# pascalPost/turbomesh

Hardware: AMD Instinct MI355X
Metric: nodes smoothed/sec (elliptic sweeps, 4096^2 blocks) + achieved HBM GB/s (higher is better)
Workload: dtype f64

## Files before the change

turbomesh_amd/csrc/tm_api.cpp:

```cpp
#include "tm_smoother.hpp"
#include <cmath>
#include <cstdlib>
#include <cstring>
#include <limits>
#include <memory>

using namespace tmh;

#include "tm_api_util.hpp"
#include "tm_ilu.hpp"
#include "tm_refine.hpp"
#include "tm_quality_dev.hpp"

static void require_gfx950() {
    static int checked = 0;
    if (checked) return;
    int dev = 0;
    HIPCHK(hipGetDevice(&dev));
    hipDeviceProp_t prop;
    HIPCHK(hipGetDeviceProperties(&prop, dev));
    if (std::strncmp(prop.gcnArchName, "gfx950", 6) != 0)
        throw TmError(TM_E_HIP, std::string("libtm_hip is built for gfx950 (MI355X) only, found ") + prop.gcnArchName);
    checked = 1;
}
// ... 596 lines not shown
            shape[4 * l + 2] = L[l].ci;
            shape[4 * l + 3] = L[l].cj;
        }
        if (cycle) {
            cycle[0] = h.nu_pre;
            cycle[1] = h.nu_post;
            cycle[2] = h.nu_coarsest;
            cycle[3] = m.mg_dirichlet ? 1 : 0;
            cycle[4] = m.mg_perimeter_step ? 1 : 0;
            cycle[5] = m.mg_perimeter_sweeps;
        }
        if (omega) *omega = h.omega;
        return TM_OK;
    });
}
int tm_smoother_precondition_probe(tm_smoother* s, const double* f, double* z, double* f_after) {
    return guarded([&]() {
        if (!s || !f || !z) throw TmError(TM_E_ARG, "null argument");
        s->impl.precondition_probe_host(f, z, f_after);
        return TM_OK;
    });
}

int tm_smoother_queue_ordering(const tm_smoother* s) { return s ? s->impl.queue_ordering : static_cast<int>(TM_E_ARG); }

int tm_smooth_mesh(const tm_mesh_desc* mesh, uint64_t iterations, const tm_solver_opt* opt, const tm_control_fn* cf, tm_stats* stats) {
    tm_smoother* h = nullptr;
    int rc = tm_smoother_create(mesh, opt, cf, nullptr, nullptr, &h);
    if (rc < 0) return rc;
    tm_stats st;
    std::memset(&st, 0, sizeof(st));
    rc = tm_smoother_iterate(h, iterations, &st);
    if (rc >= 0 && iterations > 0) {
        const int rd = tm_smoother_download(h, mesh);
        if (rd < 0) rc = rd;
    }
    tm_smoother_destroy(h);
    if (stats) *stats = st;
    return rc;
}

int tm_plan_local(const tm_mesh_desc* mesh, const int32_t* owner, int32_t rank, int32_t nranks, tm_plan_local_info* out) {
    return guarded([&]() {
        if (!mesh || !owner || !out) throw TmError(TM_E_ARG, "null argument");
        std::memset(out, 0, sizeof(*out));
        const Topology t = topo_of(mesh);
// ... 184 lines not shown
```

turbomesh_amd/csrc/tm_kernels.h:

```cpp
#pragma once
#include <hip/hip_runtime.h>
#include <cstdint>
#include "tm_edge_types.h"
#include <vector>

namespace tmh {

enum ApplyMode : int {
    MODE_RAW = 0,
    MODE_SCALED = 1,
    MODE_RESID = 2,
    MODE_RELAX = 3,
    MODE_DIAG_COPY = 4,
    MODE_DIAG_SUM9 = 5,
    MODE_DIAG_NOSTORE = 6,
    MODE_DIAG_NOLOAD = 7,
    MODE_DIAG_MATH = 8,
    MODE_MG_RESID = 9,
    MODE_MG_SMOOTH = 10,
    MODE_MG_FIRST2 = 11
};
enum DotMode : int {
    DOT_NONE = 0,
    DOT_AUX = 1,
// ... 205 lines not shown
};
hipError_t launch_white(const WhiteArgs& w, int update, hipStream_t stream);

struct MgPair {
    int nif, njf, nic, njc;
    int ci, cj;
};
hipError_t launch_mg_inject(const double2* fine, double2* coarse, const MgPair& g, double scale_x, double scale_y, hipStream_t stream);
hipError_t launch_mg_restrict(const double2* r_fine, const double2* X_coarse, double2* f_coarse, const MgPair& g, hipStream_t stream);
hipError_t launch_mg_prolong_smooth(const ApplyBlock& a, const MgPair& g, hipStream_t stream);
struct MgPairArgs {
    const double2* in = nullptr;
    const double2* xk = nullptr;
    const double2* pq = nullptr;
    const double2* f = nullptr;
    double2* out = nullptr;
    double2* out2 = nullptr;
    const double2* coarse = nullptr;
    const double2* xc = nullptr;
    double2* fc = nullptr;
    int nic = 0, njc = 0, ci = 0, cj = 0;
    int ni = 0, nj = 0;
    double omega = 1.0;
};
bool mg_pair_supported(int ni, int nj);
bool mg_pair_restrict_supported(int ni, int nj, int ci, int cj);
hipError_t launch_mg_pair(const MgPairArgs& a, int kind, hipStream_t stream);
hipError_t launch_mg_prolong_add(const double2* e_coarse, double2* e_fine, const MgPair& g, hipStream_t stream);
hipError_t launch_mg_scale(const double2* f, double2* out, int ni, int nj, double omega, hipStream_t stream);

hipError_t launch_soa_planes(const double2* in, double* plane0, double* plane1, int ni, int nj, hipStream_t stream);

hipError_t launch_debug_white_math(const double* x, const double* y, uint64_t n, double* out_acos, double* out_atan2, hipStream_t stream);

}
```

turbomesh_amd/csrc/tm_kernels.hip:

```cpp
#include "tm_kernels.h"
#include "tm_devutil.hpp"
#include "tm_refmath.h"
#include <cstdlib>
#include <type_traits>

namespace tmh {

__device__ __forceinline__ double lane_prev(double edge, double v) {
    int2 o = __builtin_bit_cast(int2, edge), s = __builtin_bit_cast(int2, v), r;
    r.x = __builtin_amdgcn_update_dpp(o.x, s.x, 0x138 , 0xf, 0xf, false);
    r.y = __builtin_amdgcn_update_dpp(o.y, s.y, 0x138, 0xf, 0xf, false);
    return __builtin_bit_cast(double, r);
}
__device__ __forceinline__ double lane_next(double edge, double v) {
    int2 o = __builtin_bit_cast(int2, edge), s = __builtin_bit_cast(int2, v), r;
    r.x = __builtin_amdgcn_update_dpp(o.x, s.x, 0x130 , 0xf, 0xf, false);
    r.y = __builtin_amdgcn_update_dpp(o.y, s.y, 0x130, 0xf, 0xf, false);
    return __builtin_bit_cast(double, r);
}
__device__ __forceinline__ double2 lane_prev(double2 edge, double2 v) { return make_double2(lane_prev(edge.x, v.x), lane_prev(edge.y, v.y)); }
__device__ __forceinline__ double2 lane_next(double2 edge, double2 v) { return make_double2(lane_next(edge.x, v.x), lane_next(edge.y, v.y)); }

__device__ __forceinline__ double2 lane_prev0(double2 v) {
    int4 s = __builtin_bit_cast(int4, v), r;
// ... 985 lines not shown
template <bool HAS_PQ>
__device__ __forceinline__ double2 mg_scaled_row(const MgMetric& g, const Row3& m, const Row3& c, const Row3& p, double P, double Q) {
    double ax = p.c.x + m.c.x, ay = p.c.y + m.c.y;
    double bx = c.h.x, by = c.h.y;
    if (HAS_PQ) {
        const double hP = 0.5 * P, hQ = 0.5 * Q;
        ax = fma(hP, p.c.x - m.c.x, ax);
        ay = fma(hP, p.c.y - m.c.y, ay);
        bx = fma(hQ, c.e.x, bx);
        by = fma(hQ, c.e.y, by);
    }
    const double kx = p.e.x - m.e.x;
    const double ky = p.e.y - m.e.y;
    double sx = g.G22 * ax, sy = g.G22 * ay;
    sx = fma(g.G11, bx, sx);
    sy = fma(g.G11, by, sy);
    sx = fma(g.m2D, c.c.x, sx);
    sy = fma(g.m2D, c.c.y, sy);
    sx = fma(g.mhG12, kx, sx);
    sy = fma(g.mhG12, ky, sy);
    return make_double2(sx * g.rinv, sy * g.rinv);
}

template <int KIND, bool HAS_PQ, bool PRO, bool RST, int U>
__device__ __forceinline__ void mg_pair_strip(const MgPairArgs& a, const Relax2Tile& t) {
    static_assert(!RST || KIND == 1, "the restriction rides behind the residual");
    const int ni = a.ni, nj = a.nj;
    const int cc = min(max(t.c, 0), nj - 1);
    const double2 zero = make_double2(0.0, 0.0);
    auto at = [&](int row) { return static_cast<size_t>(min(max(row, 0), ni - 1)) * nj + cc; };
    const bool perim_col = (t.c <= 0) || (t.c >= nj - 1);
    const bool col_in = (t.c >= 1) && (t.c <= nj - 2);
    const int nrows = t.i1 - t.i0;
    const __amdgpu_buffer_rsrc_t out_rsrc = __builtin_amdgcn_make_buffer_rsrc(a.out + static_cast<size_t>(t.i0) * nj, 0, nrows * nj * 16, 0x00020000);
    const __amdgpu_buffer_rsrc_t out2_rsrc =
        __builtin_amdgcn_make_buffer_rsrc((KIND == 1 ? a.out2 : a.out) + static_cast<size_t>(t.i0) * nj, 0, nrows * nj * 16, 0x00020000);
    const unsigned lane_off = static_cast<unsigned>(cc) * 16u;
    const int cj1 = PRO ? min(a.cj ? ((cc + 1) >> 1) : cc, a.njc - 1) : 0;
    const bool midway = PRO && a.cj && (cc & 1);

    struct Ld {
        double2 in, x, f, pq, c0, c1;
    };
    auto load_step = [&](int i, Ld& L) {
        const size_t ar = at(i + 2), aq = at(i + 1);
        L.in = a.in[ar];
        L.x = a.xk[ar];
        if (KIND == 0) L.f = a.f[aq];
        if (HAS_PQ) L.pq = a.pq[aq];
        if (PRO) {
            const int r = min(max(i + 2, 0), ni - 1);
            const int ci0 = min(a.ci ? (r >> 1) : r, a.nic - 1), ci1 = min(a.ci ? ((r + 1) >> 1) : r, a.nic - 1);
            const double2* r0 = a.coarse + static_cast<size_t>(ci0) * a.njc;
            const double2* r1 = a.coarse + static_cast<size_t>(ci1) * a.njc;
            L.c0 = r0[cj1];
            L.c1 = r1[cj1];
        }
    };
    auto entering = [&](int row, const Ld& L) {
        if (KIND == 1) return (col_in && row >= 1 && row <= ni - 2) ? L.in : zero;
        if (!PRO) return L.in;
        const double2 l0 = lane_prev0(L.c0), l1 = lane_prev0(L.c1);
        const double2 a0 = midway ? l0 : L.c0, a1 = midway ? l1 : L.c1;
        const double2 v = make_double2(L.in.x + 0.25 * ((a0.x + L.c0.x) + (a1.x + L.c1.x)), L.in.y + 0.25 * ((a0.y + L.c0.y) + (a1.y + L.c1.y)));
        return (col_in && row >= 1 && row <= ni - 2) ? v : L.in;
    };
    auto det_of = [&](double2 x) { return sub2(lane_next0(x), lane_prev0(x)); };

    Row3 A[3], S[3];
    double2 Xc[3], Xe_cur;
    MgMetric Mp = {0.0, 0.0, 0.0, 0.0, 0.0, 0.0};
    double2 f_prev = zero, pq_prev = zero;
    double2 rm2 = zero, rm1 = zero;
    Ld cur[U], nxt[U];
    {
        Ld w0, w1;
        load_step(t.i0 - 4, w0);
        load_step(t.i0 - 3, w1);
#pragma unroll
        for (int u = 0; u < U; ++u) load_step(t.i0 - 2 + u, cur[u]);
        A[0] = make_row(entering(t.i0 - 2, w0));
        A[1] = make_row(entering(t.i0 - 1, w1));
        Xc[0] = w0.x;
        Xc[1] = w1.x;
        Xe_cur = det_of(w1.x);
        A[2].c = A[2].e = A[2].h = zero;
        S[0] = S[1] = S[2] = A[2];
        Xc[2] = zero;
    }
    const int nsteps = nrows + (RST ? 3 : 2);
    auto group = [&](const int tb) {
#pragma unroll
        for (int u = 0; u < U; ++u) load_step(t.i0 - 2 + tb + U + u, nxt[u]);
#pragma unroll
        for (int u = 0; u < U; ++u) {
            const int A0 = u % 3, A1 = (u + 1) % 3, A2 = (u + 2) % 3;
            const Ld& L = cur[u];
            const int i = t.i0 - 2 + tb + u;
            const int q = i + 1;
            A[A2] = make_row(entering(i + 2, L));
            Xc[A2] = L.x;
            const double2 Xe_next = det_of(L.x);
            const MgMetric M = mg_metric(sub2(Xc[A2], Xc[A0]), Xe_cur);
            const double2 t1 = mg_scaled_row<HAS_PQ>(M, A[A0], A[A1], A[A2], HAS_PQ ? L.pq.x : 0.0, HAS_PQ ? L.pq.y : 0.0);
            const double2 fq = (KIND == 0) ? L.f : A[A1].c;
            double2 s1;
            if (KIND == 0) {
                const double2 res = sub2(fq, t1);
                s1 = make_double2(fma(a.omega, res.x, A[A1].c.x), fma(a.omega, res.y, A[A1].c.y));
            } else {
                s1 = make_double2(a.omega * fma(-a.omega, t1.x, 2.0 * A[A1].c.x), a.omega * fma(-a.omega, t1.y, 2.0 * A[A1].c.y));
            }
            const bool perim_row = (q <= 0) || (q >= ni - 1);
            if (perim_row || perim_col) s1 = zero;
            if (KIND == 1) {
                const bool own = t.out_lane && !perim_row && (q >= t.i0) && (q < t.i1);
                __builtin_amdgcn_raw_buffer_store_b128(__builtin_bit_cast(v4i32, s1), out_rsrc,
                                                       static_cast<int>(own ? lane_off + static_cast<unsigned>((q - t.i0) * nj * 16) : OOB_VOFFSET), 0, 0);
            }
            S[A2] = make_row(s1);
            const double2 t2 = mg_scaled_row<HAS_PQ>(Mp, S[A0], S[A1], S[A2], HAS_PQ ? pq_prev.x : 0.0, HAS_PQ ? pq_prev.y : 0.0);
// ... 19 lines not shown
                        acc.y = fma(wi * 0.25, l.y, acc.y);
                        acc.x = fma(wi * 0.5, v.x, acc.x);
                        acc.y = fma(wi * 0.5, v.y, acc.y);
                        acc.x = fma(wi * 0.25, r.x, acc.x);
                        acc.y = fma(wi * 0.25, r.y, acc.y);
                    };
                    row_sum(rm2, 0.25);
                    row_sum(rm1, 0.5);
                    row_sum(oz, 0.25);
                    const int ci = (i - 1) >> 1, cj = t.c >> 1, lane = t.c - t.c0 + 2;
                    const bool emit = !(t.c & 1) && lane >= 4 && lane <= 60 && t.c >= 2 && t.c <= nj - 2 && ci >= 1 && ci <= a.nic - 2 && cj <= a.njc - 2;
                    if (emit) {
                        const size_t oc = static_cast<size_t>(ci) * a.njc + cj;
                        const double2 xp = a.xc[oc + a.njc], xm = a.xc[oc - a.njc], xr = a.xc[oc + 1], xl = a.xc[oc - 1];
                        const double dxx = xp.x - xm.x, dxy = xp.y - xm.y, dex = xr.x - xl.x, dey = xr.y - xl.y;
                        const double aic = -0.5 * (fma(dxx, dxx, dxy * dxy) + fma(dex, dex, dey * dey));
                        const double k = 16.0 / ((aic == 0.0) ? 1.0 : aic);
                        a.fc[oc] = make_double2(k * acc.x, k * acc.y);
                    }
                }
                rm2 = rm1;
                rm1 = oz;
            }
            Mp = M;
            f_prev = fq;
            if (HAS_PQ) pq_prev = L.pq;
            Xe_cur = Xe_next;
        }
#pragma unroll
        for (int u = 0; u < U; ++u) cur[u] = nxt[u];
    };
    group(0);
    for (int tb = U; tb < nsteps; tb += U) group(tb);
}

template <int KIND, bool HAS_PQ, bool PRO, bool RST = false>
__global__ __launch_bounds__(256) void k_mg_pair(MgPairArgs a, int RI, int nSG, int nRC) {
    const int lane = threadIdx.x & 63;
    const int wave = threadIdx.x >> 6;
    const int total = nSG * nRC, bid = blockIdx.x;
    const int q8 = total >> 3, rem = total & 7, xcd = bid & 7, k8 = bid >> 3;
    const int logical = (xcd < rem) ? xcd * (q8 + 1) + k8 : rem * (q8 + 1) + (xcd - rem) * q8 + k8;
    const int rc = logical / nSG;
    const int sg = logical - rc * nSG;
    Relax2Tile t;
    t.c0 = (sg * 4 + wave) * (RST ? MG_RST_W : 60);
    t.c = t.c0 - 2 + lane;
    t.out_lane = (lane >= (RST ? 3 : 2)) && (lane <= (RST ? 60 : 61)) && (t.c >= 1) && (t.c <= a.nj - 2);
    t.i0 = 1 + rc * RI;
    t.i1 = min(t.i0 + RI, a.ni - 1);
    if (t.c0 + (RST ? 1 : 0) <= a.nj - 2 && t.i0 < t.i1) mg_pair_strip<KIND, HAS_PQ, PRO, RST, 3>(a, t);
}

bool mg_pair_supported(int ni, int nj) { return ni >= 5 && nj >= 5 && nj <= (1 << 20); }
bool mg_pair_restrict_supported(int ni, int nj, int ci, int cj) {
    if (!mg_pair_supported(ni, nj) || !ci || !cj) return false;
    const int nstrips = (nj - 2 + MG_RST_W - 1) / MG_RST_W, nSG = (nstrips + 3) / 4;
    return static_cast<long>(nSG) * ((ni - 2 + 17) / 18) >= 1024;
}
hipError_t launch_mg_pair(const MgPairArgs& a, int kind, hipStream_t st) {
    if (!mg_pair_supported(a.ni, a.nj)) return hipErrorInvalidValue;
    if (kind == 1 && a.fc) {
        if (!mg_pair_restrict_supported(a.ni, a.nj, a.ci, a.cj) || !a.xc) return hipErrorInvalidValue;
        const int nstrips = (a.nj - 2 + MG_RST_W - 1) / MG_RST_W, nSG = (nstrips + 3) / 4, RI = 18, nRC = (a.ni - 2 + RI - 1) / RI;
        const dim3 grid(nSG * nRC), block(256);
        if (a.pq) hipLaunchKernelGGL((k_mg_pair<1, true, false, true>), grid, block, 0, st, a, RI, nSG, nRC);
        else hipLaunchKernelGGL((k_mg_pair<1, false, false, true>), grid, block, 0, st, a, RI, nSG, nRC);
        return hipGetLastError();
    }
    const int nstrips = (a.nj - 1 + 59) / 60, nSG = (nstrips + 3) / 4, interior = a.ni - 2;
    int RI = 18;
    while (RI > 3 && static_cast<long>(nSG) * ((interior + RI - 1) / RI) < 1024) RI -= 3;
    RI = std::max(1, std::min(RI, interior));
    const int nRC = (interior + RI - 1) / RI;
    const dim3 grid(nSG * nRC), block(256);
    const bool pq = a.pq != nullptr, pro = a.coarse != nullptr;
    if (kind == 1) {
        if (pq) hipLaunchKernelGGL((k_mg_pair<1, true, false>), grid, block, 0, st, a, RI, nSG, nRC);
        else hipLaunchKernelGGL((k_mg_pair<1, false, false>), grid, block, 0, st, a, RI, nSG, nRC);
    } else if (pro) {
        if (pq) hipLaunchKernelGGL((k_mg_pair<0, true, true>), grid, block, 0, st, a, RI, nSG, nRC);
        else hipLaunchKernelGGL((k_mg_pair<0, false, true>), grid, block, 0, st, a, RI, nSG, nRC);
    } else {
        if (pq) hipLaunchKernelGGL((k_mg_pair<0, true, false>), grid, block, 0, st, a, RI, nSG, nRC);
// ... 1616 lines not shown
```

turbomesh_amd/csrc/tm_multigrid.cpp:

```cpp
#include "tm_multigrid.hpp"
#include "tm_smoother.hpp"

#include <algorithm>
#include <cmath>
#include <cstdio>
#include <cstdlib>

namespace tmh {

#define HIPCHK(x) hip_check((x), #x)

static void log_aspect_stats(const double* xy, int ni, int nj, double& mean, double& sdev) {
    mean = sdev = 0.0;
    if (!xy || ni < 3 || nj < 3) return;
    const int si = std::max(1, (ni - 2) / 64), sj = std::max(1, (nj - 2) / 64);
    double sum = 0.0, sum2 = 0.0;
    long cnt = 0;
    for (int i = 1; i < ni - 1; i += si)
        for (int j = 1; j < nj - 1; j += sj) {
            const double* c = xy + 2 * (static_cast<size_t>(i) * nj + j);
            const double ax = c[2 * nj] - c[-2 * nj], ay = c[2 * nj + 1] - c[-2 * nj + 1];
            const double bx = c[2] - c[-2], by = c[3] - c[-1];
            const double g11 = ax * ax + ay * ay, g22 = bx * bx + by * by;
            if (g11 > 0.0 && g22 > 0.0) {
// ... 105 lines not shown
    a.aux = f;
    a.out = out;
    a.ni = l.ni;
    a.nj = l.nj;
    a.omega = omega;
    a.partials = nullptr;
    HIPCHK(launch_apply_block(a, MODE_MG_SMOOTH, DOT_NONE, st));
}

void BlockMG::residual(const MgLevel& l, const double2* f, const double2* in, double2* out, hipStream_t st) const {
    ApplyBlock a;
    a.in = in;
    a.xk = l.X;
    a.pq = l.PQ;
    a.aux = f;
    a.out = out;
    a.ni = l.ni;
    a.nj = l.nj;
    a.omega = 0.0;
    a.partials = nullptr;
    HIPCHK(launch_apply_block(a, MODE_MG_RESID, DOT_NONE, st));
}

void BlockMG::vcycle(const double2* f0, double2* z, double2* w0, double2* w1, hipStream_t st) {
    const size_t nl = L.size();
    std::vector<double2*> cur(nl, nullptr), oth(nl, nullptr);
    std::vector<const double2*> rhs(nl, nullptr);
    const int pre_extra = nu_pre > 0 ? nu_pre - 1 : 0;
    auto pair_ok = [&](size_t l) { return use_pair && mg_pair_supported(L[l].ni, L[l].nj); };
    const bool pair_pre0 = pair_ok(0) && nu_pre == 2 && nl > 1, pair_post0 = pair_ok(0) && nu_post == 2;
    (void)pair_pre0;
    const int flips0 = (nl == 1) ? pre_extra + nu_coarsest : pre_extra + (pair_post0 ? 1 : nu_post);
    cur[0] = (flips0 % 2 == 0) ? z : w0;
    oth[0] = (flips0 % 2 == 0) ? w0 : z;
    rhs[0] = f0;
    L[0].r = w1;
    for (size_t l = 1; l < nl; ++l) {
        cur[l] = L[l].a;
        oth[l] = L[l].b;
        rhs[l] = L[l].f;
    }
    auto sweeps = [&](size_t l, int n) {
        for (int k = 0; k < n; ++k) {
            smooth(L[l], rhs[l], cur[l], oth[l], st);
            std::swap(cur[l], oth[l]);
        }
    };
    for (size_t l = 0; l < nl; ++l) {
// ... 51 lines not shown
            sweeps(l, nu_coarsest);
            break;
        }
        residual(L[l], rhs[l], cur[l], L[l].r, st);
        HIPCHK(launch_mg_restrict(L[l].r, L[l + 1].X, L[l + 1].f, pair(l), st));
    }
    for (size_t l = nl - 1; l-- > 0;) {
        if (nu_post == 2 && pair_ok(l)) {
            MgPairArgs a;
            a.in = cur[l];
            a.xk = L[l].X;
            a.pq = L[l].PQ;
            a.f = rhs[l];
            a.out = oth[l];
            a.coarse = cur[l + 1];
            const MgPair g = pair(l);
            a.nic = g.nic;
            a.njc = g.njc;
            a.ci = g.ci;
            a.cj = g.cj;
            a.ni = L[l].ni;
            a.nj = L[l].nj;
            a.omega = omega;
            HIPCHK(launch_mg_pair(a, 0, st));
            std::swap(cur[l], oth[l]);
            continue;
        }
        if (fuse_prolong && nu_post >= 1 && static_cast<int64_t>(L[l].ni) * L[l].nj >= fuse_prolong_min) {
            ApplyBlock a;
            a.in = cur[l];
            a.in2 = cur[l + 1];
            a.xk = L[l].X;
            a.pq = L[l].PQ;
            a.aux = rhs[l];
            a.out = oth[l];
            a.ni = L[l].ni;
            a.nj = L[l].nj;
            a.omega = omega;
            a.partials = nullptr;
            HIPCHK(launch_mg_prolong_smooth(a, pair(l), st));
            std::swap(cur[l], oth[l]);
            sweeps(l, nu_post - 1);
        } else {
            HIPCHK(launch_mg_prolong_add(cur[l + 1], cur[l], pair(l), st));
            sweeps(l, nu_post);
        }
// ... 6 lines not shown
```

turbomesh_amd/csrc/tm_multigrid.hpp:

```cpp
#pragma once
#include "tm_kernels.h"
#include <vector>

namespace tmh {

class DeviceArena;

struct MgLevel {
    int ni = 0, nj = 0;
    int ci = 0, cj = 0;
    double2 *X = nullptr, *PQ = nullptr;
    double2 *f = nullptr, *a = nullptr, *b = nullptr, *r = nullptr;
};

class BlockMG {
   public:
    int nu_pre = 2, nu_post = 2, nu_coarsest = 8;
    int64_t fuse_prolong_min = 262144;
    bool fuse_prolong = true;
    double omega = 0.8;
    bool fuse_restrict = true;
    bool use_pair = true;
    void build(DeviceArena& arena, int ni, int nj, bool has_pq, double aspect, bool worst_case);
    static double aspect_of(const double* xy, int ni, int nj);
    static double aspect_spread_of(const double* xy, int ni, int nj);
    void set_field(const double2* X0, const double2* PQ0, hipStream_t stream);
    void vcycle(const double2* f, double2* z, double2* w0, double2* w1, hipStream_t stream);
    size_t nlevels() const { return L.size(); }
    const std::vector<MgLevel>& levels() const { return L; }

   private:
    std::vector<MgLevel> L;
    void smooth(const MgLevel& l, const double2* f, const double2* in, double2* out, hipStream_t st) const;
    void residual(const MgLevel& l, const double2* f, const double2* in, double2* out, hipStream_t st) const;
    MgPair pair(size_t fine) const;
};

}
```

turbomesh_amd/csrc/tm_smoother.cpp:

```cpp
#include "tm_smoother.hpp"
#include "tm_api_util.hpp"
#include "tm_ilu.hpp"
#include "tm_refine.hpp"
#include "tm_quality_dev.hpp"
#include <algorithm>
#include <atomic>
#include <chrono>
#include <cmath>
#include <cstdio>
#include <cstdlib>
#include <cstring>
#include <map>
#include <unordered_map>

namespace tmh {

void hip_check(hipError_t e, const char* what) {
    if (e != hipSuccess) throw TmError(TM_E_HIP, std::string(what) + ": " + hipGetErrorString(e));
}
#define HIPCHK(x) hip_check((x), #x)

std::atomic<int> g_multirank_handles{0};
tm_log_fn g_log_sink = nullptr;
void* g_log_ctx = nullptr;
// ... 430 lines not shown
            border_ids.push_back(static_cast<const int32_t*>(upload_table(ids.data(), ids.size() * 4)));
        }
        poff2_edge = off2;
        nwg_apply2 = off2 + edge_nf.nwg;
    }
    pipelined_single = fuse_pairs && !(has_hooks && (lp.send_ids.size() > 0 || !lp.ghost_gid.empty())) && edge_nf.nrows > 0 && lp.n_owned >= (1 << 21);
    if (const char* e = std::getenv("TM_SINGLE_PIPELINED")) pipelined_single = pipelined_single && std::atoi(e) != 0;
    fuse_triples = fuse_pairs && edge_nf.nrows == 0 && !(has_hooks && (!lp.send_ids.empty() || !lp.ghost_gid.empty()));
    if (const char* e = std::getenv("TM_FUSE_3")) fuse_triples = fuse_triples && std::atoi(e) != 0;
    if (fuse_triples || triples_coupled) {
        poff3.clear();
        rows3.clear();
        int off3 = 0;
        rows3 = relax3_rows_of_owned_blocks();
        for (size_t k = 0; k < lp.owned_blocks.size(); ++k) {
            const int64_t b = lp.owned_blocks[k];
            const int bi = static_cast<int>(topo.ni[b]), bj = static_cast<int>(topo.nj[b]);
            if (!relax3_supported(bi, bj)) fuse_triples = false;
            poff3.push_back(off3);
            off3 += relax3_block_nwg(bi, bj, rows3[k]);
        }
        nwg_apply3 = off3;
    }
    nwg_vec = vec_nwg(n_owned);
    const int nwg3_all = fuse_triples ? nwg_apply3 : (triples_coupled ? nwg_apply3 + std::max(edge_L[2].nwg, fused_levels.nstrips) : 0);
    if (vk_overlap) {
        int off_ov = 0;
        for (int64_t b : lp.owned_blocks) {
            poff_ov.push_back(off_ov);
            off_ov += apply_block_nwg_overlap(static_cast<int>(topo.ni[b]), static_cast<int>(topo.nj[b]), apply_rows);
        }
        poff_edge_ov = off_ov;
        nwg_apply_ov = off_ov + edge.nwg;
    }
    if (vk_able && std::max(nwg_apply, nwg_apply_ov) <= 512) nwg_vec = std::min(nwg_vec, 512);
    lazy = !has_hooks && opt.inner != TM_INNER_RELAX && std::max(std::max(nwg_apply, nwg_apply_ov), nwg_vec) <= 512 && !(opt.flags & TM_OPT_EAGER_SCALARS);
    const int nwg_refine = refine() ? csr_nwg(n_owned) : 0;
    const uint64_t npart = static_cast<uint64_t>(std::max(std::max(std::max(std::max(std::max(nwg_apply, nwg_apply_ov), nwg_apply2), nwg3_all), nwg_vec), nwg_refine)) * MAX_PARTIALS;
    fuse_s = !has_hooks && opt.inner == TM_INNER_BICGSTAB && !(opt.flags & TM_OPT_EAGER_SCALARS);
    fuse_p = fuse_s;
    if (const char* e = std::getenv("TM_FUSE_P")) fuse_p = fuse_p && std::atoi(e) != 0;
    fuse2 = fuse_p;
    if (const char* e = std::getenv("TM_FUSE_2")) fuse2 = fuse2 && std::atoi(e) != 0;
    if (fuse_p) {
        p_alt = vec();
        v_alt = vec();
    }
    if (fuse2) r_alt = vec();
    const int rows = static_cast<int>(npart / MAX_PARTIALS);
    const struct {
        const char* what;
        int nwg;
    } producers[] = {{"operator", nwg_apply},
                     {"operator (overlapping strips)", nwg_apply_ov},
                     {"sweep pairs", nwg_apply2},
                     {"sweep triples", nwg3_all},
                     {"vector kernels", nwg_vec},
                     {"GMRES Gram-Schmidt", (opt.inner == TM_INNER_GMRES || reference()) ? vec_nwg(n_owned) : 0},
                     {"perimeter-row right-hand side", opt.inner != TM_INNER_RELAX ? edge.nwg : 0},
                     {"refinement step", nwg_refine}};
    if (std::getenv("TM_DEBUG_RUNS"))
        std::fprintf(stderr, "[tm] partial-sum rows: %d allocated; operator %d, overlapping strips %d, pairs %d, triples %d, vector kernels %d (vec_nwg %d)\n", rows,
                     nwg_apply, nwg_apply_ov, nwg_apply2, nwg3_all, nwg_vec, vec_nwg(n_owned));
    for (const auto& q : producers)
        if (q.nwg > rows)
            throw TmError(TM_E_HIP, std::string("internal: the ") + q.what + " launch has " + std::to_string(q.nwg) + " workgroups, the partial-sum buffer " +
                                        std::to_string(rows) + " rows");
    return npart;
}

void Smoother::alloc_reductions(uint64_t npart) {
    partials_guard = false;
    if (const char* e = std::getenv("TM_PARTIALS_GUARD")) partials_guard = std::atoi(e) != 0;
    const uint64_t nguard = partials_guard ? GUARD_DOUBLES : 0;
    for (int k = 0; k < (lazy ? 3 : 1); ++k) part_buf[k] = arena.alloc_n<double>(npart + nguard);
    partials = part_buf[0];
    red = arena.alloc_n<double>(MAX_PARTIALS + nguard);
    if (partials_guard) {
        for (int k = 0; k < 3; ++k) guard[k] = part_buf[k] ? part_buf[k] + npart : nullptr;
        guard[3] = red ? red + MAX_PARTIALS : nullptr;
    }
    S_buf[0] = arena.alloc_n<KrylovScalars>(1);
    S_buf[1] = lazy ? arena.alloc_n<KrylovScalars>(1) : S_buf[0];
// ... 319 lines not shown
}

void Smoother::white_launch(int update) {
    WhiteArgs w;
    const auto idx = [&](int64_t b) { return lp.local_start[std::lower_bound(lp.owned_blocks.begin(), lp.owned_blocks.end(), b) - lp.owned_blocks.begin()]; };
    w.x0 = X + idx(0);
    w.x1 = X + idx(1);
    w.pq0 = PQ + idx(0);
    w.pq1 = PQ + idx(1);
    w.ni0 = static_cast<int>(topo.ni[0]);
    w.nj0 = static_cast<int>(topo.nj[0]);
    w.ni1 = static_cast<int>(topo.ni[1]);
    w.nj1 = static_cast<int>(topo.nj[1]);
    w.le_p0 = static_cast<int>(white_le.position[0]);
    w.le_p1 = static_cast<int>(white_le.position[1]);
    w.le_fi0 = static_cast<int>(white_le.first_internal[0]);
    w.le_fi1 = static_cast<int>(white_le.first_internal[1]);
    w.le_dir0 = static_cast<int>(white_le.direction[0]);
    w.ds_target = cf.ds_target;
    w.theta_target = cf.theta_target;
    HIPCHK(launch_white(w, update, stream));
}

void Smoother::precondition(const double2* in, double2* out) {
    double2* const in_w = const_cast<double2*>(in);
    const size_t nb = lp.owned_blocks.size(), ns = mg_streams.size();
    auto dims = [&](size_t k, int& bi, int& bj) {
        const int64_t b = lp.owned_blocks[k];
        bi = static_cast<int>(topo.ni[b]);
        bj = static_cast<int>(topo.nj[b]);
    };
    int bi, bj;
    if (mg_dirichlet)
        for (size_t k = 0; k < nb; ++k) {
            dims(k, bi, bj);
            const int64_t ls = lp.local_start[k];
            HIPCHK(launch_ring_dirichlet(in_w + ls, X + ls, PQ ? PQ + ls : nullptr, t + ls, bi, bj, stream));
        }
    if (ns > 1) HIPCHK(hipEventRecord(mg_fork, stream));
    for (size_t k = 0; k < nb; ++k) {
        const int64_t ls = lp.local_start[k];
        hipStream_t q = ns > 1 ? mg_streams[k % ns] : stream;
        if (ns > 1 && k < ns) HIPCHK(hipStreamWaitEvent(q, mg_fork, 0));
        mg[k].vcycle(in + ls, out + ls, mg_w0 + ls, mg_w1 + ls, q);
    }
    for (size_t q = 0; q < ns && ns > 1; ++q) {
        HIPCHK(hipEventRecord(mg_join[q], mg_streams[q]));
        HIPCHK(hipStreamWaitEvent(stream, mg_join[q], 0));
    }
    for (size_t k = 0; k < nb; ++k) {
        dims(k, bi, bj);
        const int64_t ls = lp.local_start[k];
        if (mg_dirichlet) HIPCHK(launch_ring_restore(in_w + ls, t + ls, bi, bj, stream));
        if (!mg_perimeter_step) HIPCHK(launch_copy_perimeter(in + ls, out + ls, bi, bj, stream));
    }
    if (!mg_perimeter_step) return;
    for (int sweep = 0; sweep < mg_perimeter_sweeps; ++sweep) {
        if (has_hooks) {
            exchange(out);
            exchange_finish();
        }
        HIPCHK(launch_edge_rows(edge, out, X, PQ, nullptr, t, 0.0, MODE_SCALED, DOT_NONE, nullptr, stream));
        for (size_t k = 0; k < lp.owned_blocks.size(); ++k) {
            const int64_t b = lp.owned_blocks[k];
            const int64_t ls = lp.local_start[k];
            HIPCHK(launch_perimeter_sub(in + ls, t + ls, out + ls, static_cast<int>(topo.ni[b]), static_cast<int>(topo.nj[b]), stream));
        }
    }
}

void Smoother::precondition_probe_host(const double* f, double* z, double* f_after) {
    if (!use_mg) throw TmError(TM_E_UNSUPPORTED, "tm_smoother_precondition_probe needs a handle created with TM_INNER_MG_BICGSTAB");
    if (has_hooks) throw TmError(TM_E_UNSUPPORTED, "tm_smoother_precondition_probe is available on single-process handles only");
    for (size_t k = 0; k < lp.owned_blocks.size(); ++k) mg[k].set_field(X + lp.local_start[k], PQ ? PQ + lp.local_start[k] : nullptr, stream);
    HIPCHK(hipMemcpyAsync(p, f, sizeof(double2) * n_owned, hipMemcpyHostToDevice, stream));
    precondition(p, p_hat);
    HIPCHK(hipMemcpyAsync(z, p_hat, sizeof(double2) * n_owned, hipMemcpyDeviceToHost, stream));
    if (f_after) HIPCHK(hipMemcpyAsync(f_after, p, sizeof(double2) * n_owned, hipMemcpyDeviceToHost, stream));
    sync();
}

int Smoother::poll_done(uint64_t it, bool final) {
    auto verdict = [&](const KrylovScalars* h, uint64_t at) {
        if (h->done[0] && h->done[1]) return (h->done[0] == 1 && h->done[1] == 1) ? 1 : 2;
        bool progress = false;
        for (int c = 0; c < 2; ++c) {
            if (h->done[c]) continue;
            if (!(stall_best[c] > 0.0) || h->rr[c] < 0.25 * stall_best[c]) {
                stall_best[c] = h->rr[c];
                progress = true;
            }
        }
        if (progress) stall_since = at;
        else if (at > stall_since && at - stall_since > stall_window) {
            stalled = true;
            return 2;
        }
        return 0;
    };
    flush_pending();
    if (!pipelined_poll) {
        HIPCHK(hipMemcpyAsync(h_S, S, sizeof(KrylovScalars), hipMemcpyDeviceToHost, stream));
// ... 67 lines not shown
                apply_virtual(VK_R, r, v, t, p_alt, v_alt, p, r_alt, U);
                std::swap(r, r_alt);
                std::swap(p, p_alt);
                std::swap(v, v_alt);
                apply_virtual(VK_S2, r, v, nullptr, nullptr, t);
                st.operator_sweeps += 2;
                it_total += 1;
                if (it_total % opt.check_every == 0 || it_total == opt.max_inner) {
                    const int verdict = poll_done(it_total, it_total == opt.max_inner);
                    if (verdict) {
                        converged = verdict == 1;
                        breakdown = !converged;
                        break;
                    }
                }
                continue;
            }
            if (fuse_p) {
                apply_virtual(VK_P, r, p, v, p_alt, v_alt);
                std::swap(p, p_alt);
                std::swap(v, v_alt);
            } else {
                HIPCHK(launch_p_update(scalars_for(), r, p, v, n_owned, nwg_vec, stream));
                if (use_mg) {
                    precondition(p, p_hat);
                    apply(p_hat, v, MODE_SCALED, DOT_AUX, r_hat, X, 0.0, STEP_SIGMA);
                } else {
                    apply(p, v, MODE_SCALED, DOT_AUX, r_hat, X, 0.0, STEP_SIGMA);
                }
            }
            if (fuse_s) {
                apply_virtual(VK_S, r, v, nullptr, nullptr, t);
                HIPCHK(launch_xr_update_vs(scalars_for(), U, p, v, t, r, r_hat, n_owned, nwg_vec, partials, stream));
                reduce_update(nwg_vec, STEP_RHO);
                st.operator_sweeps += 2;
                it_total += 1;
                if (it_total % opt.check_every == 0 || it_total == opt.max_inner) {
                    const int verdict = poll_done(it_total, it_total == opt.max_inner);
                    if (verdict) {
                        converged = verdict == 1;
                        breakdown = !converged;
                        break;
                    }
                }
                continue;
            }
            HIPCHK(launch_s_update(scalars_for(), r, v, s, n_owned, nwg_vec, partials, stream));
            reduce_update(nwg_vec, STEP_SS);
            if (use_mg) {
                precondition(s, s_hat);
                apply(s_hat, t, MODE_SCALED, DOT_AUX2, s, X, 0.0, STEP_TSTT);
            } else {
                apply(s, t, MODE_SCALED, DOT_IN, nullptr, X, 0.0, STEP_TSTT);
            }
            HIPCHK(launch_xr_update(scalars_for(), U, use_mg ? p_hat : p, use_mg ? s_hat : s, s, t, r, r_hat, n_owned, nwg_vec, partials, stream));
            reduce_update(nwg_vec, STEP_RHO);
            st.operator_sweeps += 2;
            it_total += 1;
            if (it_total % opt.check_every == 0 || it_total == opt.max_inner) {
                const int verdict = poll_done(it_total, it_total == opt.max_inner);
                if (verdict) {
                    converged = verdict == 1;
                    breakdown = !converged;
                    break;
                }
            }
        }
        if (fuse2) {
            flush_pending();
            HIPCHK(launch_xr_update_vs(scalars_for(), U, p, v, t, r, r_hat, n_owned, nwg_vec, partials, stream));
        }
        if (converged || !breakdown || stalled || restarts >= 8 || it_total >= opt.max_inner) break;
// ... 943 lines not shown
```

turbomesh_amd/csrc/tm_smoother.hpp:

```cpp
#pragma once
#include "../../include/tm_hip.h"
#include <cstdlib>
#include "tm_edge_tables.hpp"
#include "tm_kernels.h"
#include "tm_multigrid.hpp"
#include "tm_plan.hpp"
#include <cmath>
#include <atomic>
#include <memory>
#include <string>
#include <functional>
#include <vector>

namespace tmh {

struct TmError : std::runtime_error {
    int code;
    TmError(int c, const std::string& m) : std::runtime_error(m), code(c) {}
};
void hip_check(hipError_t e, const char* what);
extern std::atomic<int> g_multirank_handles;
extern tm_log_fn g_log_sink;
extern void* g_log_ctx;

// ... 26 lines not shown
    Topology topo;
    std::vector<PlanRow> all_rows;
    LocalPlan lp;
    tm_solver_opt opt{};
    tm_control_fn cf{};
    tm_comm_hooks hooks{};
    bool has_hooks = false;
    std::vector<int32_t> owner;
    hipStream_t stream = nullptr;
    DeviceArena arena;

    int64_t n_owned = 0, n_local = 0, n_ghost = 0, dof_global = 0;
    double2 *X = nullptr, *U = nullptr, *r = nullptr, *r_hat = nullptr, *p = nullptr, *v = nullptr, *s = nullptr, *t = nullptr;
    double2 *PQ = nullptr, *tmpA = nullptr, *tmpB = nullptr;
    double2 *p_hat = nullptr, *s_hat = nullptr, *mg_w0 = nullptr, *mg_w1 = nullptr;
    std::vector<BlockMG> mg;
    bool use_mg = false;
    bool mg_perimeter_step = false;
    bool mg_dirichlet = false;
    std::vector<hipStream_t> mg_streams;
    std::vector<hipEvent_t> mg_join;
    hipEvent_t mg_fork = nullptr;
    int mg_perimeter_sweeps = 2;
    void precondition(const double2* in, double2* out);
    void precondition_probe_host(const double* f, double* z, double* f_after);
    double2* M = nullptr;
    double2* M2 = nullptr;
    bool fuse_pairs = false;
    bool relax2_store_nt = true;
    bool pair_sync_events = false;
    size_t inside_lds = 0;
    EdgeRowsDev edge;
    std::vector<double> h_rhs;
    struct RhsTable {
        double* dev = nullptr;
        std::vector<const double*> src;
    };
    std::vector<RhsTable> rhs_tables;
    EdgeRowsDev edge_nf;
    EdgeRowsDev edge_nf_g;
    std::vector<int> dyn_mask;
    std::vector<const int32_t*> border_ids;
    std::vector<int> border_n;
    void prefill_fixed();
    double* partials = nullptr;
    double* red = nullptr;
    KrylovScalars* S = nullptr;
// ... 196 lines not shown
```

Baseline: 447.5 billion.

## Fold the scaled operator application and dot into the last multigrid post-smoothing pair

The final fine-level post-smoothing pair kernel now also applies the scaled operator to the freshly smoothed correction. It writes v/t and accumulates the DOT_AUX/AUX2 partial sums in the same strip pass, with a third row of lag. The perimeter rows are handled by an edge-rows launch, and one reduction covers both. This removes a separate full-grid read of z and write of v per BiCGSTAB half-step. The cost is heavier per-strip register use, narrower strips, and a gating condition on block size and hierarchy shape.

```diff
diff --git a/turbomesh_amd/csrc/tm_api.cpp b/turbomesh_amd/csrc/tm_api.cpp
--- a/turbomesh_amd/csrc/tm_api.cpp
+++ b/turbomesh_amd/csrc/tm_api.cpp
@@ -642,6 +642,16 @@
     });
 }
 
+#ifdef TM_DEBUG_EXPORTS
+int tm_debug_mg_fold_probe(tm_smoother* s, int branch, int folded, const double* f, const double* aux, double* z, double* v, double* sums) {
+    return guarded([&]() {
+        if (!s || !f || !aux || !z || !v || !sums || branch < 0 || branch > 1) throw TmError(TM_E_ARG, "bad argument");
+        s->impl.fold_probe_host(branch, folded != 0, f, aux, z, v, sums);
+        return TM_OK;
+    });
+}
+#endif
+
 int tm_smoother_queue_ordering(const tm_smoother* s) { return s ? s->impl.queue_ordering : static_cast<int>(TM_E_ARG); }
 
 int tm_smooth_mesh(const tm_mesh_desc* mesh, uint64_t iterations, const tm_solver_opt* opt, const tm_control_fn* cf, tm_stats* stats) {
diff --git a/turbomesh_amd/csrc/tm_kernels.h b/turbomesh_amd/csrc/tm_kernels.h
--- a/turbomesh_amd/csrc/tm_kernels.h
+++ b/turbomesh_amd/csrc/tm_kernels.h
@@ -251,8 +251,13 @@
     int nic = 0, njc = 0, ci = 0, cj = 0;
     int ni = 0, nj = 0;
     double omega = 1.0;
+    double2* vout = nullptr;
+    const double2* aux = nullptr;
+    double* partials = nullptr;
+    int dot = DOT_NONE;
 };
 bool mg_pair_supported(int ni, int nj);
+int mg_pair_apply_nwg(int ni, int nj);
 bool mg_pair_restrict_supported(int ni, int nj, int ci, int cj);
 hipError_t launch_mg_pair(const MgPairArgs& a, int kind, hipStream_t stream);
 hipError_t launch_mg_prolong_add(const double2* e_coarse, double2* e_fine, const MgPair& g, hipStream_t stream);
diff --git a/turbomesh_amd/csrc/tm_kernels.hip b/turbomesh_amd/csrc/tm_kernels.hip
--- a/turbomesh_amd/csrc/tm_kernels.hip
+++ b/turbomesh_amd/csrc/tm_kernels.hip
@@ -1031,9 +1031,11 @@
     return make_double2(sx * g.rinv, sy * g.rinv);
 }
 
-template <int KIND, bool HAS_PQ, bool PRO, bool RST, int U>
-__device__ __forceinline__ void mg_pair_strip(const MgPairArgs& a, const Relax2Tile& t) {
+template <int KIND, bool HAS_PQ, bool PRO, bool RST, int A3, int U>
+__device__ __forceinline__ void mg_pair_strip(const MgPairArgs& a, const Relax2Tile& t, double (&acc)[MAX_PARTIALS]) {
     static_assert(!RST || KIND == 1, "the restriction rides behind the residual");
+    static_assert(!A3 || (KIND == 0 && (A3 == DOT_AUX || A3 == DOT_AUX2)), "the operator application rides behind the post-sweeps");
+    constexpr int H = A3 ? 3 : 2;
     const int ni = a.ni, nj = a.nj;
     const int cc = min(max(t.c, 0), nj - 1);
     const double2 zero = make_double2(0.0, 0.0);
@@ -1044,12 +1046,15 @@
     const __amdgpu_buffer_rsrc_t out_rsrc = __builtin_amdgcn_make_buffer_rsrc(a.out + static_cast<size_t>(t.i0) * nj, 0, nrows * nj * 16, 0x00020000);
     const __amdgpu_buffer_rsrc_t out2_rsrc =
         __builtin_amdgcn_make_buffer_rsrc((KIND == 1 ? a.out2 : a.out) + static_cast<size_t>(t.i0) * nj, 0, nrows * nj * 16, 0x00020000);
+    const __amdgpu_buffer_rsrc_t v_rsrc =
+        __builtin_amdgcn_make_buffer_rsrc((A3 ? a.vout : a.out) + static_cast<size_t>(t.i0) * nj, 0, nrows * nj * 16, 0x00020000);
     const unsigned lane_off = static_cast<unsigned>(cc) * 16u;
     const int cj1 = PRO ? min(a.cj ? ((cc + 1) >> 1) : cc, a.njc - 1) : 0;
     const bool midway = PRO && a.cj && (cc & 1);
 
     struct Ld {
         double2 in, x, f, pq, c0, c1;
+        double2 aux;
     };
     auto load_step = [&](int i, Ld& L) {
         const size_t ar = at(i + 2), aq = at(i + 1);
@@ -1057,6 +1062,7 @@
         L.x = a.xk[ar];
         if (KIND == 0) L.f = a.f[aq];
         if (HAS_PQ) L.pq = a.pq[aq];
+        if (A3) L.aux = a.aux[at(i - 1)];
         if (PRO) {
             const int r = min(max(i + 2, 0), ni - 1);
             const int ci0 = min(a.ci ? (r >> 1) : r, a.nic - 1), ci1 = min(a.ci ? ((r + 1) >> 1) : r, a.nic - 1);
@@ -1076,36 +1082,37 @@
     };
     auto det_of = [&](double2 x) { return sub2(lane_next0(x), lane_prev0(x)); };
 
-    Row3 A[3], S[3];
+    Row3 A[3], S[3], Z[3];
     double2 Xc[3], Xe_cur;
-    MgMetric Mp = {0.0, 0.0, 0.0, 0.0, 0.0, 0.0};
-    double2 f_prev = zero, pq_prev = zero;
+    MgMetric Mp = {0.0, 0.0, 0.0, 0.0, 0.0, 0.0}, Mpp = Mp;
+    double2 f_prev = zero, pq_prev = zero, pq_pp = zero;
     double2 rm2 = zero, rm1 = zero;
     Ld cur[U], nxt[U];
     {
         Ld w0, w1;
-        load_step(t.i0 - 4, w0);
-        load_step(t.i0 - 3, w1);
-#pragma unroll
-        for (int u = 0; u < U; ++u) load_step(t.i0 - 2 + u, cur[u]);
-        A[0] = make_row(entering(t.i0 - 2, w0));
-        A[1] = make_row(entering(t.i0 - 1, w1));
+        load_step(t.i0 - H - 2, w0);
+        load_step(t.i0 - H - 1, w1);
+#pragma unroll
+        for (int u = 0; u < U; ++u) load_step(t.i0 - H + u, cur[u]);
+        A[0] = make_row(entering(t.i0 - H, w0));
+        A[1] = make_row(entering(t.i0 - H + 1, w1));
         Xc[0] = w0.x;
         Xc[1] = w1.x;
         Xe_cur = det_of(w1.x);
         A[2].c = A[2].e = A[2].h = zero;
         S[0] = S[1] = S[2] = A[2];
+        Z[0] = Z[1] = Z[2] = A[2];
         Xc[2] = zero;
     }
-    const int nsteps = nrows + (RST ? 3 : 2);
+    const int nsteps = nrows + (A3 ? 4 : (RST ? 3 : 2));
     auto group = [&](const int tb) {
 #pragma unroll
-        for (int u = 0; u < U; ++u) load_step(t.i0 - 2 + tb + U + u, nxt[u]);
+        for (int u = 0; u < U; ++u) load_step(t.i0 - H + tb + U + u, nxt[u]);
 #pragma unroll
         for (int u = 0; u < U; ++u) {
             const int A0 = u % 3, A1 = (u + 1) % 3, A2 = (u + 2) % 3;
             const Ld& L = cur[u];
-            const int i = t.i0 - 2 + tb + u;
+            const int i = t.i0 - H + tb + u;
             const int q = i + 1;
             A[A2] = make_row(entering(i + 2, L));
             Xc[A2] = L.x;
@@ -1171,6 +1178,17 @@
                 rm2 = rm1;
                 rm1 = oz;
             }
+            if (A3) {
+                const double2 zi = (col_in && i >= 1 && i <= ni - 2) ? o : f_prev;
+                Z[A2] = make_row(zi);
+                const double2 t3 = mg_scaled_row<HAS_PQ>(Mpp, Z[A0], Z[A1], Z[A2], HAS_PQ ? pq_pp.x : 0.0, HAS_PQ ? pq_pp.y : 0.0);
+                const bool own = t.out_lane && (i - 1 >= t.i0) && (i - 1 < t.i1);
+                __builtin_amdgcn_raw_buffer_store_b128(__builtin_bit_cast(v4i32, t3), v_rsrc,
+                                                       static_cast<int>(own ? lane_off + static_cast<unsigned>((i - 1 - t.i0) * nj * 16) : OOB_VOFFSET), 0, 2);
+                accumulate<A3>(acc, zero, own ? t3 : zero, L.aux);
+                Mpp = Mp;
+                if (HAS_PQ) pq_pp = pq_prev;
+            }
             Mp = M;
             f_prev = fq;
             if (HAS_PQ) pq_prev = L.pq;
@@ -1183,8 +1201,9 @@
     for (int tb = U; tb < nsteps; tb += U) group(tb);
 }
 
-template <int KIND, bool HAS_PQ, bool PRO, bool RST = false>
+template <int KIND, bool HAS_PQ, bool PRO, bool RST = false, int A3 = 0>
 __global__ __launch_bounds__(256) void k_mg_pair(MgPairArgs a, int RI, int nSG, int nRC) {
+    constexpr bool W58 = RST || A3 != 0;
     const int lane = threadIdx.x & 63;
     const int wave = threadIdx.x >> 6;
     const int total = nSG * nRC, bid = blockIdx.x;
@@ -1193,12 +1212,14 @@
     const int rc = logical / nSG;
     const int sg = logical - rc * nSG;
     Relax2Tile t;
-    t.c0 = (sg * 4 + wave) * (RST ? MG_RST_W : 60);
+    t.c0 = (sg * 4 + wave) * (W58 ? MG_RST_W : 60);
     t.c = t.c0 - 2 + lane;
-    t.out_lane = (lane >= (RST ? 3 : 2)) && (lane <= (RST ? 60 : 61)) && (t.c >= 1) && (t.c <= a.nj - 2);
+    t.out_lane = (lane >= (W58 ? 3 : 2)) && (lane <= (W58 ? 60 : 61)) && (t.c >= 1) && (t.c <= a.nj - 2);
     t.i0 = 1 + rc * RI;
     t.i1 = min(t.i0 + RI, a.ni - 1);
-    if (t.c0 + (RST ? 1 : 0) <= a.nj - 2 && t.i0 < t.i1) mg_pair_strip<KIND, HAS_PQ, PRO, RST, 3>(a, t);
+    double acc[MAX_PARTIALS] = {0.0, 0.0, 0.0, 0.0};
+    if (t.c0 + (W58 ? 1 : 0) <= a.nj - 2 && t.i0 < t.i1) mg_pair_strip<KIND, HAS_PQ, PRO, RST, A3, 3>(a, t, acc);
+    if (A3) block_partials<256, dot_columns(A3)>(acc, a.partials + static_cast<size_t>(logical) * MAX_PARTIALS);
 }
 
 bool mg_pair_supported(int ni, int nj) { return ni >= 5 && nj >= 5 && nj <= (1 << 20); }
@@ -1207,8 +1228,30 @@
     const int nstrips = (nj - 2 + MG_RST_W - 1) / MG_RST_W, nSG = (nstrips + 3) / 4;
     return static_cast<long>(nSG) * ((ni - 2 + 17) / 18) >= 1024;
 }
+static void mg_pair_apply_grid(int ni, int nj, int& RI, int& nSG, int& nRC) {
+    const int nstrips = (nj - 2 + MG_RST_W - 1) / MG_RST_W, interior = ni - 2;
+    nSG = (nstrips + 3) / 4;
+    RI = 18;
+    while (RI > 3 && static_cast<long>(nSG) * ((interior + RI - 1) / RI) < 1024) RI -= 3;
+    RI = std::max(1, std::min(RI, interior));
+    nRC = (interior + RI - 1) / RI;
+}
+int mg_pair_apply_nwg(int ni, int nj) {
+    int RI, nSG, nRC;
+    mg_pair_apply_grid(ni, nj, RI, nSG, nRC);
+    return nSG * nRC;
+}
 hipError_t launch_mg_pair(const MgPairArgs& a, int kind, hipStream_t st) {
     if (!mg_pair_supported(a.ni, a.nj)) return hipErrorInvalidValue;
+    if (a.vout) {
+        if (kind != 0 || a.pq || !a.coarse || !a.aux || !a.partials || (a.dot != DOT_AUX && a.dot != DOT_AUX2)) return hipErrorInvalidValue;
+        int RI, nSG, nRC;
+        mg_pair_apply_grid(a.ni, a.nj, RI, nSG, nRC);
+        const dim3 grid(nSG * nRC), block(256);
+        if (a.dot == DOT_AUX) hipLaunchKernelGGL((k_mg_pair<0, false, true, false, DOT_AUX>), grid, block, 0, st, a, RI, nSG, nRC);
+        else hipLaunchKernelGGL((k_mg_pair<0, false, true, false, DOT_AUX2>), grid, block, 0, st, a, RI, nSG, nRC);
+        return hipGetLastError();
+    }
     if (kind == 1 && a.fc) {
         if (!mg_pair_restrict_supported(a.ni, a.nj, a.ci, a.cj) || !a.xc) return hipErrorInvalidValue;
         const int nstrips = (a.nj - 2 + MG_RST_W - 1) / MG_RST_W, nSG = (nstrips + 3) / 4, RI = 18, nRC = (a.ni - 2 + RI - 1) / RI;
diff --git a/turbomesh_amd/csrc/tm_multigrid.cpp b/turbomesh_amd/csrc/tm_multigrid.cpp
--- a/turbomesh_amd/csrc/tm_multigrid.cpp
+++ b/turbomesh_amd/csrc/tm_multigrid.cpp
@@ -151,8 +151,13 @@
     HIPCHK(launch_apply_block(a, MODE_MG_RESID, DOT_NONE, st));
 }
 
-void BlockMG::vcycle(const double2* f0, double2* z, double2* w0, double2* w1, hipStream_t st) {
+bool BlockMG::apply_fold_supported() const {
+    return use_pair && nu_pre == 2 && nu_post == 2 && L.size() > 2 && mg_pair_supported(L[0].ni, L[0].nj);
+}
+
+void BlockMG::vcycle(const double2* f0, double2* z, double2* w0, double2* w1, hipStream_t st, const MgApplyFold* fold) {
     const size_t nl = L.size();
+    if (fold && !apply_fold_supported()) throw TmError(TM_E_ARG, "internal: this hierarchy cannot apply the operator behind its cycle");
     std::vector<double2*> cur(nl, nullptr), oth(nl, nullptr);
     std::vector<const double2*> rhs(nl, nullptr);
     const int pre_extra = nu_pre > 0 ? nu_pre - 1 : 0;
@@ -250,6 +255,12 @@
             a.ni = L[l].ni;
             a.nj = L[l].nj;
             a.omega = omega;
+            if (fold && l == 0) {
+                a.vout = fold->v;
+                a.aux = fold->aux;
+                a.partials = fold->partials;
+                a.dot = fold->dot;
+            }
             HIPCHK(launch_mg_pair(a, 0, st));
             std::swap(cur[l], oth[l]);
             continue;
diff --git a/turbomesh_amd/csrc/tm_multigrid.hpp b/turbomesh_amd/csrc/tm_multigrid.hpp
--- a/turbomesh_amd/csrc/tm_multigrid.hpp
+++ b/turbomesh_amd/csrc/tm_multigrid.hpp
@@ -13,6 +13,13 @@
     double2 *f = nullptr, *a = nullptr, *b = nullptr, *r = nullptr;
 };
 
+struct MgApplyFold {
+    double2* v;
+    const double2* aux;
+    double* partials;
+    int dot;
+};
+
 class BlockMG {
    public:
     int nu_pre = 2, nu_post = 2, nu_coarsest = 8;
@@ -25,7 +32,8 @@
     static double aspect_of(const double* xy, int ni, int nj);
     static double aspect_spread_of(const double* xy, int ni, int nj);
     void set_field(const double2* X0, const double2* PQ0, hipStream_t stream);
-    void vcycle(const double2* f, double2* z, double2* w0, double2* w1, hipStream_t stream);
+    void vcycle(const double2* f, double2* z, double2* w0, double2* w1, hipStream_t stream, const MgApplyFold* fold = nullptr);
+    bool apply_fold_supported() const;
     size_t nlevels() const { return L.size(); }
     const std::vector<MgLevel>& levels() const { return L; }
 
diff --git a/turbomesh_amd/csrc/tm_smoother.cpp b/turbomesh_amd/csrc/tm_smoother.cpp
--- a/turbomesh_amd/csrc/tm_smoother.cpp
+++ b/turbomesh_amd/csrc/tm_smoother.cpp
@@ -476,6 +476,30 @@
         }
         nwg_apply3 = off3;
     }
+    mg_fold_apply = false;
+    nwg_fold = 0;
+    if (use_mg && !has_hooks && !white && !mg_perimeter_step && !mg_dirichlet && edge_nf.nrows == 0 && !mg.empty()) {
+        int64_t fold_min = int64_t(1) << 23, smallest = INT64_MAX;
+        if (const char* e = std::getenv("TM_MG_FOLD_MIN_NODES")) fold_min = std::atoll(e);
+        bool able = true;
+        for (size_t k = 0; k < lp.owned_blocks.size(); ++k) {
+            const int64_t b = lp.owned_blocks[k];
+            able = able && mg[k].apply_fold_supported();
+            smallest = std::min<int64_t>(smallest, topo.ni[b] * topo.nj[b]);
+        }
+        mg_fold_apply = able && smallest >= fold_min;
+        if (const char* e = std::getenv("TM_MG_FOLD")) mg_fold_apply = able && (std::atoi(e) & 1) != 0;
+    }
+    if (mg_fold_apply) {
+        fold_poff.clear();
+        int offf = 0;
+        for (int64_t b : lp.owned_blocks) {
+            fold_poff.push_back(offf);
+            offf += mg_pair_apply_nwg(static_cast<int>(topo.ni[b]), static_cast<int>(topo.nj[b]));
+        }
+        fold_poff_edge = offf;
+        nwg_fold = offf + edge.nwg;
+    }
     nwg_vec = vec_nwg(n_owned);
     const int nwg3_all = fuse_triples ? nwg_apply3 : (triples_coupled ? nwg_apply3 + std::max(edge_L[2].nwg, fused_levels.nstrips) : 0);
     if (vk_overlap) {
@@ -488,9 +512,9 @@
         nwg_apply_ov = off_ov + edge.nwg;
     }
     if (vk_able && std::max(nwg_apply, nwg_apply_ov) <= 512) nwg_vec = std::min(nwg_vec, 512);
-    lazy = !has_hooks && opt.inner != TM_INNER_RELAX && std::max(std::max(nwg_apply, nwg_apply_ov), nwg_vec) <= 512 && !(opt.flags & TM_OPT_EAGER_SCALARS);
+    lazy = !has_hooks && opt.inner != TM_INNER_RELAX && std::max(std::max(std::max(nwg_apply, nwg_apply_ov), nwg_vec), nwg_fold) <= 512 && !(opt.flags & TM_OPT_EAGER_SCALARS);
     const int nwg_refine = refine() ? csr_nwg(n_owned) : 0;
-    const uint64_t npart = static_cast<uint64_t>(std::max(std::max(std::max(std::max(std::max(nwg_apply, nwg_apply_ov), nwg_apply2), nwg3_all), nwg_vec), nwg_refine)) * MAX_PARTIALS;
+    const uint64_t npart = static_cast<uint64_t>(std::max(std::max(std::max(std::max(std::max(std::max(nwg_apply, nwg_apply_ov), nwg_apply2), nwg3_all), nwg_vec), nwg_refine), nwg_fold)) * MAX_PARTIALS;
     fuse_s = !has_hooks && opt.inner == TM_INNER_BICGSTAB && !(opt.flags & TM_OPT_EAGER_SCALARS);
     fuse_p = fuse_s;
     if (const char* e = std::getenv("TM_FUSE_P")) fuse_p = fuse_p && std::atoi(e) != 0;
@@ -512,7 +536,8 @@
                      {"vector kernels", nwg_vec},
                      {"GMRES Gram-Schmidt", (opt.inner == TM_INNER_GMRES || reference()) ? vec_nwg(n_owned) : 0},
                      {"perimeter-row right-hand side", opt.inner != TM_INNER_RELAX ? edge.nwg : 0},
-                     {"refinement step", nwg_refine}};
+                     {"refinement step", nwg_refine},
+                     {"cycle with the operator behind it", nwg_fold}};
     if (std::getenv("TM_DEBUG_RUNS"))
         std::fprintf(stderr, "[tm] partial-sum rows: %d allocated; operator %d, overlapping strips %d, pairs %d, triples %d, vector kernels %d (vec_nwg %d)\n", rows,
                      nwg_apply, nwg_apply_ov, nwg_apply2, nwg3_all, nwg_vec, vec_nwg(n_owned));
@@ -878,7 +903,7 @@
     HIPCHK(launch_white(w, update, stream));
 }
 
-void Smoother::precondition(const double2* in, double2* out) {
+void Smoother::precondition(const double2* in, double2* out, double2* vout, const double2* aux, int dot) {
     double2* const in_w = const_cast<double2*>(in);
     const size_t nb = lp.owned_blocks.size(), ns = mg_streams.size();
     auto dims = [&](size_t k, int& bi, int& bj) {
@@ -898,6 +923,11 @@
         const int64_t ls = lp.local_start[k];
         hipStream_t q = ns > 1 ? mg_streams[k % ns] : stream;
         if (ns > 1 && k < ns) HIPCHK(hipStreamWaitEvent(q, mg_fork, 0));
+        if (vout) {
+            const MgApplyFold fold = {vout + ls, aux + ls, partials + static_cast<size_t>(fold_poff[k]) * MAX_PARTIALS, dot};
+            mg[k].vcycle(in + ls, out + ls, mg_w0 + ls, mg_w1 + ls, q, &fold);
+            continue;
+        }
         mg[k].vcycle(in + ls, out + ls, mg_w0 + ls, mg_w1 + ls, q);
     }
     for (size_t q = 0; q < ns && ns > 1; ++q) {
@@ -923,6 +953,12 @@
             HIPCHK(launch_perimeter_sub(in + ls, t + ls, out + ls, static_cast<int>(topo.ni[b]), static_cast<int>(topo.nj[b]), stream));
         }
     }
+}
+
+void Smoother::precondition_apply(const double2* in, double2* out, double2* vout, int dot, const double2* aux, int step) {
+    precondition(in, out, vout, aux, dot);
+    HIPCHK(launch_edge_rows(edge, out, X, PQ, aux, vout, 0.0, MODE_SCALED, dot, partials + static_cast<size_t>(fold_poff_edge) * MAX_PARTIALS, stream));
+    reduce_update(nwg_fold, step);
 }
 
 void Smoother::precondition_probe_host(const double* f, double* z, double* f_after) {
@@ -934,6 +970,29 @@
     HIPCHK(hipMemcpyAsync(z, p_hat, sizeof(double2) * n_owned, hipMemcpyDeviceToHost, stream));
     if (f_after) HIPCHK(hipMemcpyAsync(f_after, p, sizeof(double2) * n_owned, hipMemcpyDeviceToHost, stream));
     sync();
+}
+
+void Smoother::fold_probe_host(int branch, bool folded, const double* f, const double* aux, double* z, double* vout, double* sums) {
+    if (!use_mg || has_hooks) throw TmError(TM_E_UNSUPPORTED, "the fold probe needs a single-process handle created with TM_INNER_MG_BICGSTAB");
+    if (folded && !mg_fold_apply) throw TmError(TM_E_UNSUPPORTED, "this handle does not apply the operator inside its cycles (TM_MG_FOLD, DESIGN.md section 5)");
+    const int dot = branch == 0 ? DOT_AUX : DOT_AUX2;
+    flush_pending();
+    for (size_t k = 0; k < lp.owned_blocks.size(); ++k) mg[k].set_field(X + lp.local_start[k], PQ ? PQ + lp.local_start[k] : nullptr, stream);
+    HIPCHK(hipMemcpyAsync(p, f, sizeof(double2) * n_owned, hipMemcpyHostToDevice, stream));
+    HIPCHK(hipMemcpyAsync(s, aux, sizeof(double2) * n_owned, hipMemcpyHostToDevice, stream));
+    if (folded) {
+        precondition(p, p_hat, v, s, dot);
+        HIPCHK(launch_edge_rows(edge, p_hat, X, PQ, s, v, 0.0, MODE_SCALED, dot, partials + static_cast<size_t>(fold_poff_edge) * MAX_PARTIALS, stream));
+        reduce(nwg_fold);
+    } else {
+        precondition(p, p_hat);
+        apply(p_hat, v, MODE_SCALED, dot, s, X, 0.0, -1);
+    }
+    HIPCHK(hipMemcpyAsync(h_red, red, sizeof(double) * MAX_PARTIALS, hipMemcpyDeviceToHost, stream));
+    HIPCHK(hipMemcpyAsync(z, p_hat, sizeof(double2) * n_owned, hipMemcpyDeviceToHost, stream));
+    HIPCHK(hipMemcpyAsync(vout, v, sizeof(double2) * n_owned, hipMemcpyDeviceToHost, stream));
+    sync();
+    for (int k = 0; k < 4; ++k) sums[k] = (branch == 0 && k >= 2) ? 0.0 : h_red[k];
 }
 
 int Smoother::poll_done(uint64_t it, bool final) {
@@ -1047,7 +1106,9 @@
                 std::swap(v, v_alt);
             } else {
                 HIPCHK(launch_p_update(scalars_for(), r, p, v, n_owned, nwg_vec, stream));
-                if (use_mg) {
+                if (use_mg && mg_fold_apply && !profile) {
+                    precondition_apply(p, p_hat, v, DOT_AUX, r_hat, STEP_SIGMA);
+                } else if (use_mg) {
                     precondition(p, p_hat);
                     apply(p_hat, v, MODE_SCALED, DOT_AUX, r_hat, X, 0.0, STEP_SIGMA);
                 } else {
@@ -1072,7 +1133,9 @@
             }
             HIPCHK(launch_s_update(scalars_for(), r, v, s, n_owned, nwg_vec, partials, stream));
             reduce_update(nwg_vec, STEP_SS);
-            if (use_mg) {
+            if (use_mg && mg_fold_apply && !profile) {
+                precondition_apply(s, s_hat, t, DOT_AUX2, s, STEP_TSTT);
+            } else if (use_mg) {
                 precondition(s, s_hat);
                 apply(s_hat, t, MODE_SCALED, DOT_AUX2, s, X, 0.0, STEP_TSTT);
             } else {
diff --git a/turbomesh_amd/csrc/tm_smoother.hpp b/turbomesh_amd/csrc/tm_smoother.hpp
--- a/turbomesh_amd/csrc/tm_smoother.hpp
+++ b/turbomesh_amd/csrc/tm_smoother.hpp
@@ -72,7 +72,12 @@
     std::vector<hipEvent_t> mg_join;
     hipEvent_t mg_fork = nullptr;
     int mg_perimeter_sweeps = 2;
-    void precondition(const double2* in, double2* out);
+    void precondition(const double2* in, double2* out, double2* vout = nullptr, const double2* aux = nullptr, int dot = 0);
+    bool mg_fold_apply = false;
+    std::vector<int> fold_poff;
+    int fold_poff_edge = 0, nwg_fold = 0;
+    void precondition_apply(const double2* in, double2* out, double2* vout, int dot, const double2* aux, int step);
+    void fold_probe_host(int branch, bool folded, const double* f, const double* aux, double* z, double* v, double* sums);
     void precondition_probe_host(const double* f, double* z, double* f_after);
     double2* M = nullptr;
     double2* M2 = nullptr;
```

New measurement: 447.5 billion. No clear change (-0.0%).
